# ShuangXieIrene/ssds.pytorch

Hardware: AMD Instinct MI355X
Metric: images/sec (fwd+decode+NMS) SSD-MobileNetV2@512 (higher is better)
Workload: dtype bf16

## Files before the change

### include/ssdk.h

```cpp
#ifndef SSDK_H_
#define SSDK_H_

#include <stddef.h>
#include <stdint.h>

#ifdef __cplusplus
extern "C" {
#endif

#define SSDK_VERSION 245

#define SSDK_MAX_LEVELS 8
#define SSDK_MAX_ANCHORS 16
#define SSDK_MAX_TOPN 1024
#define SSDK_MAX_NDET 1024
#define SSDK_MAX_NMS_N 8192
#define SSDK_MAX_GT 256

enum {
  SSDK_OK = 0,
  SSDK_E_BADARG = -1,
  SSDK_E_WORKSPACE = -2,
  SSDK_E_LAUNCH = -3,
  SSDK_E_NODEVICE = -4
// ... 100 lines not shown
                             int stride, int by_scale, float thr_a, float thr_b, float radius, const void* conf,
                             const void* loc, int dtype, float negpos_ratio, float beta, int loc_loss, void* d_conf,
                             void* d_loc, float* sums, void* workspace, size_t workspace_bytes, void* stream);

int ssdk_map_match(const float* scores, const float* boxes, const float* classes, int B, int D,
                   const float* targets, int G, int num_classes, float conf_threshold, float iou_threshold,
                   long long* keys, unsigned char* tp, int* npos, void* stream);

int ssdk_map_average_precision(const unsigned char* tp_sorted, const long long* seg_offsets, const int* npos,
                               int num_classes, double* ap, void* stream);

enum { SSDK_LAYOUT_NCHW = 0, SSDK_LAYOUT_NHWC = 1 };
typedef struct ssdk_conv_desc {
  const void* x;
  const void* w;
  const float* scale;
  const float* bias;
  const void* residual;
  void* y;
  void* y2;
  int32_t N, Cin, H, W, Cout, k, stride, groups;
  int32_t act, act2, split;
  int32_t dtype;
  int32_t in_layout, out_layout;
  int32_t res_mode;
  const void* w_frag;
} ssdk_conv_desc;
size_t ssdk_weight_frag_bytes(int rows, int K);
size_t ssdk_conv_workspace_bytes(int N, int Cin, int H, int W, int Cout, int k, int stride, int dtype);
int ssdk_conv(const ssdk_conv_desc* desc, void* workspace, size_t workspace_bytes, void* stream);
int ssdk_conv_sequence(const ssdk_conv_desc* descs, int n, void* workspace, size_t workspace_bytes,
                       void* stream);

typedef struct ssdk_mbconv_desc {
  const void* x;
  void* y;
  const void* w_expand;
  const float* scale_expand;
  const float* bias_expand;
  const void* w_dw;
  const void* bias_dw;
  const void* w_project;
  const float* scale_project;
  const float* bias_project;
  int32_t N, H, W, Cin, Chid, Cout, stride, residual, dtype;
  int32_t stem;
  int32_t variant;
  int32_t image_nw;
  const void* w_image;
  size_t w_image_bytes;
} ssdk_mbconv_desc;
int ssdk_mbconv(const ssdk_mbconv_desc* desc, void* stream);
size_t ssdk_mbk_image_bytes(int Cin, int Chid, int Cout, int stride, int out_width, int image_nw, int* nfo);

enum { SSDK_FUSE_SAME = 0, SSDK_FUSE_UP2 = 1, SSDK_FUSE_POOL2 = 2 };
typedef struct ssdk_fuse_desc {
  const void* a;
  const void* b;
  const void* c;
  void* y;
  float w0, w1, w2;
  int32_t mode_b, mode_c;
  int32_t N, H, W, C;
  int32_t hb, wb, hc, wc;
  int32_t dtype;
} ssdk_fuse_desc;
int ssdk_fuse(const ssdk_fuse_desc* desc, void* stream);

int ssdk_preprocess(const void* x, int src_dtype, int src_layout, int N, int H, int W, int C, const float* mean,
                    const float* std, void* y, int dst_dtype, void* stream);

typedef struct ssdk_augment_desc {
  int64_t src_offset;
  int32_t src_h, src_w;
  int32_t crop_x, crop_y, crop_w, crop_h;
  int32_t canvas_w, canvas_h, paste_x, paste_y;
  int32_t flip;
  float color[12];
  float fill[3];
} ssdk_augment_desc;
size_t ssdk_augment_desc_bytes(void);
size_t ssdk_augment_workspace_bytes(int B);
int ssdk_augment(const void* pixels, size_t pixels_bytes, const ssdk_augment_desc* descs_host, int B, int H, int W,
                 const float* mean, const float* std, void* y, int dst_dtype, void* workspace, size_t workspace_bytes,
                 void* stream);

int ssdk_pw_prepare(const float* w32, void* w16, void* wt16, int Cout, int Cin, int dtype, void* stream);
size_t ssdk_pw_stats_workspace_bytes(int B, int K, int M, int HW);
int ssdk_pw_forward_stats(const void* x, const void* a, const float* bias, void* y, float* sums, void* workspace,
                          size_t workspace_bytes, int B, int K, int M, int HW, int dtype, void* stream);
int ssdk_pw_forward(const void* x, const void* a, const float* bias, void* y, int B, int K, int M, int HW, int dtype,
                    void* stream);
size_t ssdk_pw_wgrad_workspace_bytes(int B, int Cout, int Cin, int HW);
int ssdk_pw_wgrad(const void* dy, const void* x, float* dw, void* workspace, size_t workspace_bytes, int B, int Cout, int Cin,
                  int HW, int dtype, void* stream);

int ssdk_im2col3x3(const void* x, void* col, int B, int C, int H, int W, int stride, int dtype, void* stream);
int ssdk_col2im3x3(const void* dcol, void* dx, int B, int C, int H, int W, int stride, int dtype, void* stream);
int ssdk_im2col3x3_folded(const void* x, void* col, int B, int C, int H, int W, int stride, int dtype, void* stream);
int ssdk_col2im3x3_folded(const void* dcol, void* dx, int B, int C, int H, int W, int stride, int dtype, void* stream);

size_t ssdk_stem3x3s2_wgrad_workspace_bytes(int N, int H);
int ssdk_stem3x3s2_fwd(const void* x, const float* w, void* y, int N, int Cin, int H, int W, int Cout, int dtype, void* stream);
int ssdk_stem3x3s2_wgrad(const void* x, const void* dy, float* dw, void* workspace, size_t workspace_bytes, int N, int Cin, int H, int W,
                         int Cout, int dtype, void* stream);

// ... 196 lines not shown
```

### ssds.pytorch_amd/csrc/ssdk_mbk.hip

```cpp
#include "ssdk_common.h"
#include "ssdk_flow_common.h"
#include "ssdk_scan.h"

namespace ssdk {

struct MbkParams {
  const u16* x;
  u16* y;
  const unsigned char* img;
  int N, H, W, Ho, Wo, Cin, Chid, Cout, residual;
  int pairs, halves;
  unsigned items;
  unsigned long long* dbg;
  unsigned wave_mask, pair_mask;
};

template <int KS, int NW, int NCHW, int NFO>
struct MbkGeo {
  static constexpr int NP = (NCHW + 1) / 2;
  static constexpr int PAIR_KB = 2 * KS + NFO;
  static constexpr int MISC_KB = (NCHW * 384 + 1023) / 1024;
  static constexpr int m_be = 0, m_wd = NCHW * 64, m_bd = NCHW * (64 + 288);
  static constexpr int SPB_KB = 2;
  static_assert(NFO * 128 <= SPB_KB * 1024, "projection BN block");
  __host__ __device__ static size_t weights(int halves) { return (size_t)halves * NW * NP * PAIR_KB * 1024; }
  __host__ __device__ static size_t misc_off(int halves) { return weights(halves); }
  __host__ __device__ static size_t spb_off(int halves) { return misc_off(halves) + (size_t)NW * MISC_KB * 1024; }
  __host__ __device__ static size_t bytes(int halves) { return spb_off(halves) + (size_t)halves * SPB_KB * 1024; }
};

template <int S, int NS>
struct MbkItem {
  static constexpr int NXS = NS * S;
  static constexpr int NR = S + 3;
};

template <int S, int NS, int KS, int NW, int NCHW, int NFO>
struct MbkLds {
  using G = MbkGeo<KS, NW, NCHW, NFO>;
  using I = MbkItem<S, NS>;
  static constexpr int FT = 2 * NS * NFO;
  static constexpr int XF = FT % 5 == 0 ? 5 : (FT % 8 == 0 ? 8 : 4);
  static_assert(FT % XF == 0, "exchange rounds");
  static constexpr int xt = 0;
  static constexpr int misc = xt + I::NR * I::NXS * KS * 1024;
  static constexpr int spb = misc + NW * G::MISC_KB * 1024;
  static constexpr int xch = spb + G::SPB_KB * 1024;
  static constexpr int bytes = xch + NW * XF * 1024;
};

__device__ __forceinline__ void mbk_mfma_guard() {
  __builtin_amdgcn_sched_barrier(0);
  asm volatile("s_nop 15\n\ts_nop 3" ::: "memory");
  __builtin_amdgcn_sched_barrier(0);
}
__device__ __forceinline__ void mbk_valu_guard() {
  __builtin_amdgcn_sched_barrier(0);
  asm volatile("s_nop 3" ::: "memory");
  __builtin_amdgcn_sched_barrier(0);
}
__device__ __forceinline__ u32 fl_from_left2(u32 cur, u32 prev) {
  const int old = __builtin_amdgcn_update_dpp(0, (int)prev, 0x121, 0xf, 0xf, true);
  return (u32)__builtin_amdgcn_update_dpp(old, (int)cur, 0x111, 0xf, 0xf, false);
}
__device__ __forceinline__ u32 fl_from_right2(u32 cur, u32 next) {
  const int old = __builtin_amdgcn_update_dpp(0, (int)next, 0x12f, 0xf, 0xf, true);
  return (u32)__builtin_amdgcn_update_dpp(old, (int)cur, 0x101, 0xf, 0xf, false);
}

template <int DT, int S, int NS, int KS, int NW, int NCHW, int NFO, bool DBG = false>
__global__ __launch_bounds__(64 * NW, 2) void mbk_kernel(const MbkParams p) {
  using L = MbkLds<S, NS, KS, NW, NCHW, NFO>;
  using G = MbkGeo<KS, NW, NCHW, NFO>;
  using I = MbkItem<S, NS>;
  constexpr int NR = I::NR, NXS = I::NXS, NE = NR * NXS;
  constexpr int XF = L::XF, FT = L::FT, NP = G::NP, PAIR_KB = G::PAIR_KB;
  constexpr int NO = 2 * NS;
  constexpr bool ODD = (NCHW & 1) != 0;
  constexpr int ROUNDS = FT / XF;
  extern __shared__ __attribute__((aligned(16))) unsigned char smem[];
  const u32 tid = threadIdx.x, lane = tid & 63u;
  const u32 fr = lane & 15u, fg = lane >> 4;
  const int wv = __builtin_amdgcn_readfirstlane((int)(tid >> 6));
  const int Cin = p.Cin, Cout = p.Cout, H = p.H, W = p.W, Ho = p.Ho, Wo = p.Wo;

  const u32 item = blockIdx.x;
  const int half = (int)(item % (u32)p.halves);
  const u32 rem = item / (u32)p.halves;
  const int n = (int)(rem / (u32)p.pairs), rp = (int)(rem % (u32)p.pairs);
  const int oy0 = 2 * rp;
  const int iy0 = S * oy0 - 1;
  const int co_base = half * 16 * NFO;
  const u16* ximg = p.x + (size_t)n * H * W * Cin;
  const bool stamp = p.dbg != nullptr && blockIdx.x == 0 && tid == 0;
  if (stamp) p.dbg[0] = __builtin_readcyclecounter();

  const u32x4* wimg = reinterpret_cast<const u32x4*>(p.img + ((size_t)(half * NW + wv) * NP) * ((size_t)PAIR_KB * 1024)) + lane;
  u32x4 wa[KS], wb[KS];
#pragma unroll
  for (int ks = 0; ks < KS; ++ks) {
    wa[ks] = wimg[(size_t)ks * 64];
    wb[ks] = wimg[(size_t)(KS + ks) * 64];
  }

  for (int e = wv; e < NE; e += NW) {
    const int r = e / NXS, xs = e % NXS;
    int iy = iy0 + r;
    iy = iy < 0 ? 0 : (iy > H - 1 ? H - 1 : iy);
    const int col = S == 1 ? 16 * xs + (int)fr : 2 * (16 * (xs >> 1) + (int)fr) + (xs & 1);
    const u16* src = ximg + ((size_t)iy * W + col) * Cin + fg * 8;
#pragma unroll
    for (int ks = 0; ks < KS; ++ks)
      __builtin_amdgcn_global_load_lds((glb_u8*)(src + ks * 32), (lds_u8*)(smem + L::xt + (e * KS + ks) * 1024), 16, 0, 0);
  }
  {
    const unsigned char* src = p.img + G::misc_off(p.halves) + (size_t)wv * (G::MISC_KB * 1024) + lane * 16;
#pragma unroll
    for (int k = 0; k < G::MISC_KB; ++k)
      __builtin_amdgcn_global_load_lds((glb_u8*)(src + k * 1024), (lds_u8*)(smem + L::misc + (wv * G::MISC_KB + k) * 1024), 16, 0, 0);
  }
  if (wv == 0) {
    const unsigned char* src = p.img + G::spb_off(p.halves) + (size_t)half * (G::SPB_KB * 1024) + lane * 16;
#pragma unroll
    for (int k = 0; k < G::SPB_KB; ++k)
      __builtin_amdgcn_global_load_lds((glb_u8*)(src + k * 1024), (lds_u8*)(smem + L::spb + k * 1024), 16, 0, 0);
  }
  asm volatile("s_waitcnt vmcnt(0)" ::: "memory");
  __syncthreads();
  if (stamp) p.dbg[1] = __builtin_readcyclecounter();

  fl_f2 hi[NR];
#pragma unroll
  for (int r = 0; r < NR; ++r) {
    const float k = ((unsigned)(iy0 + r) < (unsigned)H) ? kFlSixth : 0.f;
    hi[r] = fl_f2{k, k};
  }

  f32x4 yacc[NO][NFO];
#pragma unroll
  for (int o = 0; o < NO; ++o)
#pragma unroll
    for (int f = 0; f < NFO; ++f) yacc[o][f] = f32x4{0.f, 0.f, 0.f, 0.f};

  const unsigned char* xt = smem + L::xt + lane * 16;
  const unsigned char* mc = smem + L::misc + wv * (G::MISC_KB * 1024);

  auto chunk = [&](int c, const u32x4 (&w)[KS], u32 (&dout)[NO][2]) {
    const f32x4 bv = *reinterpret_cast<const f32x4*>(mc + G::m_be + (c * 4 + (int)fg) * 16);
    f32x4 e[NE];
#pragma unroll
    for (int i = 0; i < NE; ++i) e[i] = bv;
#pragma unroll
    for (int ks = 0; ks < KS; ++ks) {
      u32x4 xf[NE];
#pragma unroll
      for (int i = 0; i < NE; ++i) xf[i] = *reinterpret_cast<const u32x4*>(xt + (i * KS + ks) * 1024);
#pragma unroll
      for (int i = 0; i < NE; ++i) e[i] = fl_mfma<DT>(w[ks], xf[i], e[i]);
    }
    uint2 wt[9];
#pragma unroll
    for (int t = 0; t < 9; ++t) wt[t] = *reinterpret_cast<const uint2*>(mc + G::m_wd + ((c * 9 + t) * 4 + (int)fg) * 8);
    const uint2 bdi = *reinterpret_cast<const uint2*>(mc + G::m_bd + (c * 4 + (int)fg) * 8);
    mbk_mfma_guard();
    u32 ew[NR][NXS][2];
#pragma unroll
    for (int r = 0; r < NR; ++r)
#pragma unroll
      for (int xs = 0; xs < NXS; ++xs) {
        ew[r][xs][0] = fl_unit_pack(e[r * NXS + xs][0], e[r * NXS + xs][1], hi[r]);
        ew[r][xs][1] = fl_unit_pack(e[r * NXS + xs][2], e[r * NXS + xs][3], hi[r]);
      }
#pragma unroll
    for (int o = 0; o < 2; ++o)
#pragma unroll
      for (int j = 0; j < NS; ++j) {
        fl_h2 s[2] = {fl_as_h2(bdi.x), fl_as_h2(bdi.y)};
#pragma unroll
        for (int ky = 0; ky < 3; ++ky) {
          const int r = S * o + ky;
          const uint2 w0 = wt[ky * 3], w1 = wt[ky * 3 + 1], w2 = wt[ky * 3 + 2];
#pragma unroll
          for (int wd = 0; wd < 2; ++wd) {
            u32 tl, tc, tr;
            if constexpr (S == 1) {
              tc = ew[r][j][wd];
              tl = j == 0 ? fl_from_left(tc) : fl_from_left2(tc, ew[r][j > 0 ? j - 1 : 0][wd]);
              tr = j == NS - 1 ? fl_from_right(tc) : fl_from_right2(tc, ew[r][j < NS - 1 ? j + 1 : j][wd]);
            } else {
              const u32 odd = ew[r][2 * j + 1][wd];
              tc = ew[r][2 * j][wd];
              tl = j == 0 ? fl_from_left(odd) : fl_from_left2(odd, ew[r][j > 0 ? 2 * j - 1 : 1][wd]);
              tr = odd;
            }
            const u32 ww0 = wd ? w0.y : w0.x, ww1 = wd ? w1.y : w1.x, ww2 = wd ? w2.y : w2.x;
            s[wd] = __builtin_elementwise_fma(fl_as_h2(tl), fl_as_h2(ww0), s[wd]);
            s[wd] = __builtin_elementwise_fma(fl_as_h2(tc), fl_as_h2(ww1), s[wd]);
            if (ky == 2) s[wd] = fl_fma_clamp01(fl_as_h2(tr), fl_as_h2(ww2), s[wd]);
            else s[wd] = __builtin_elementwise_fma(fl_as_h2(tr), fl_as_h2(ww2), s[wd]);
          }
        }
        dout[o * NS + j][0] = fl_as_u32(s[0]);
        dout[o * NS + j][1] = fl_as_u32(s[1]);
      }
  };

  constexpr int FH = NFO / 2;
  for (int t = 0; t < NP; ++t) {
    const u32x4* wp = wimg + (size_t)t * (PAIR_KB * 64);
    const bool last = t == NP - 1;
    const u32x4* wn = wimg + (size_t)(last ? t : t + 1) * (PAIR_KB * 64);
    u32 d0[NO][2], d1[NO][2];
    u32x4 wf0[FH], wf1[NFO - FH];
#pragma unroll
    for (int f = 0; f < FH; ++f) wf0[f] = wp[(size_t)(2 * KS + f) * 64];
    chunk(2 * t, wa, d0);
    __builtin_amdgcn_sched_barrier(0);
    u32x4 na[KS];
#pragma unroll
    for (int ks = 0; ks < KS; ++ks) na[ks] = wn[(size_t)ks * 64];
#pragma unroll
    for (int f = FH; f < NFO; ++f) wf1[f - FH] = wp[(size_t)(2 * KS + f) * 64];
    if (!(ODD && last)) {
      chunk(2 * t + 1, wb, d1);
    } else {
#pragma unroll
      for (int o = 0; o < NO; ++o) d1[o][0] = d1[o][1] = 0u;
    }
    __builtin_amdgcn_sched_barrier(0);
    u32x4 nb[KS];
#pragma unroll
    for (int ks = 0; ks < KS; ++ks) nb[ks] = wn[(size_t)(KS + ks) * 64];
    u32x4 db[NO];
#pragma unroll
    for (int o = 0; o < NO; ++o) db[o] = u32x4{d0[o][0], d0[o][1], d1[o][0], d1[o][1]};
    if constexpr (DBG) {
      if (!((p.pair_mask >> t) & 1u) || !((p.wave_mask >> wv) & 1u)) {
#pragma unroll
        for (int o = 0; o < NO; ++o) db[o] = u32x4{0u, 0u, 0u, 0u};
      }
    }
    mbk_valu_guard();
#pragma unroll
    for (int f = 0; f < NFO; ++f)
#pragma unroll
      for (int o = 0; o < NO; ++o)
        yacc[o][f] = fl_mfma<SSDK_F16>(f < FH ? wf0[f < FH ? f : 0] : wf1[f >= FH ? f - FH : 0], db[o], yacc[o][f]);
    __builtin_amdgcn_sched_barrier(0);
#pragma unroll
    for (int ks = 0; ks < KS; ++ks) {
      wa[ks] = na[ks];
      wb[ks] = nb[ks];
    }
  }
  if (stamp) p.dbg[2] = __builtin_readcyclecounter();

  unsigned char* xb = smem + L::xch;
  const unsigned char* spb = smem + L::spb;
  constexpr int GPW = (XF + NW - 1) / NW;
  uint2 resv[ROUNDS][GPW];
#pragma unroll
  for (int R = 0; R < ROUNDS; ++R)
#pragma unroll
    for (int gg = 0; gg < GPW; ++gg) {
      const int g = wv + gg * NW, q = R * XF + g, oj = q / NFO, f = q % NFO;
      const int oy = oy0 + oj / NS, ox = 16 * (oj % NS) + (int)fr, co = co_base + f * 16 + (int)fg * 4;
      resv[R][gg] = make_uint2(0u, 0u);
      if (S == 1 && p.residual && g < XF && oy < Ho && co < Cout)
        resv[R][gg] = *reinterpret_cast<const uint2*>(ximg + ((size_t)oy * W + ox) * Cin + co);
    }
#pragma unroll
  for (int R = 0; R < ROUNDS; ++R) {
#pragma unroll
    for (int g = 0; g < XF; ++g) {
      const int q = R * XF + g, oj = q / NFO, f = q % NFO;
      *reinterpret_cast<f32x4*>(xb + ((wv * XF + g) * 64 + (int)lane) * 16) = yacc[oj][f];
    }
    __syncthreads();
#pragma unroll
    for (int gg = 0; gg < GPW; ++gg) {
      const int g = wv + gg * NW;
      if (g < XF) {
        const int q = R * XF + g, oj = q / NFO, f = q % NFO;
        f32x4 y = *reinterpret_cast<const f32x4*>(xb + ((0 * XF + g) * 64 + (int)lane) * 16);
#pragma unroll
        for (int w2 = 1; w2 < NW; ++w2) {
          const f32x4 t2 = *reinterpret_cast<const f32x4*>(xb + ((w2 * XF + g) * 64 + (int)lane) * 16);
          y = y + t2;
        }
        const int oy = oy0 + oj / NS, ox = 16 * (oj % NS) + (int)fr;
        const int co = co_base + f * 16 + (int)fg * 4;
        if (oy < Ho && co < Cout) {
          const f32x4 spv = *reinterpret_cast<const f32x4*>(spb + (f * 4 + (int)fg) * 32);
          const f32x4 bpv = *reinterpret_cast<const f32x4*>(spb + (f * 4 + (int)fg) * 32 + 16);
          u32 h01 = fl_pack2<DT>(fmaf(y[0], spv[0], bpv[0]), fmaf(y[1], spv[1], bpv[1]));
          u32 h23 = fl_pack2<DT>(fmaf(y[2], spv[2], bpv[2]), fmaf(y[3], spv[3], bpv[3]));
          if (S == 1 && p.residual) {
            const uint2 xr = resv[R][gg];
            h01 = fl_pack2<DT>(fl_from16<DT>(h01 & 0xffffu) + fl_from16<DT>(xr.x & 0xffffu), fl_from16<DT>(h01 >> 16) + fl_from16<DT>(xr.x >> 16));
            h23 = fl_pack2<DT>(fl_from16<DT>(h23 & 0xffffu) + fl_from16<DT>(xr.y & 0xffffu), fl_from16<DT>(h23 >> 16) + fl_from16<DT>(xr.y >> 16));
          }
          u16* yrow = p.y + (((size_t)n * Ho + oy) * Wo + ox) * Cout;
          *reinterpret_cast<uint2*>(yrow + co) = make_uint2(h01, h23);
        }
      }
    }
    if (R + 1 < ROUNDS) __syncthreads();
  }
  if (stamp) p.dbg[3] = __builtin_readcyclecounter();
}

template <int DT, int S, int NS, int KS, int NW, int NCHW, int NFO, bool DBG = false>
static void mbk_launch(const MbkParams& p, hipStream_t stream) {
  constexpr int lds = MbkLds<S, NS, KS, NW, NCHW, NFO>::bytes;
  static_assert(lds <= 160 * 1024, "LDS");
  (void)hipFuncSetAttribute(reinterpret_cast<const void*>(&mbk_kernel<DT, S, NS, KS, NW, NCHW, NFO, DBG>),
                            hipFuncAttributeMaxDynamicSharedMemorySize, lds);
  hipLaunchKernelGGL((mbk_kernel<DT, S, NS, KS, NW, NCHW, NFO, DBG>), dim3(p.items), dim3(64 * NW), lds, stream, p);
}

constexpr int kMbkNW = 4;
struct MbkInst {
  int s, ns, ks, nchw, nfo;
};
static const MbkInst kMbkInst[] = {{1, 1, 5, 15, 10}, {2, 1, 3, 9, 10}, {1, 2, 2, 6, 4}, {1, 2, 2, 6, 6}, {1, 2, 3, 9, 6},
                                   {2, 2, 1, 3, 4}, {1, 4, 1, 3, 2}};

static int mbk_find(int stride, int Wo, int Cin, int Chid, int Cout, int nw, int* halves) {
  if (nw != kMbkNW || Cin % 32 || Chid % 16 || Cout % 16 || Wo % 16) return -1;
  const int ks = Cin / 32, nch = Chid / 16, nchw = (nch + nw - 1) / nw, ns = Wo / 16;
  for (int i = 0; i < (int)(sizeof(kMbkInst) / sizeof(kMbkInst[0])); ++i) {
    const MbkInst& k = kMbkInst[i];
    if (k.s == stride && k.ns == ns && k.ks == ks && k.nchw == nchw && Cout % (16 * k.nfo) == 0) {
      if (halves) *halves = Cout / (16 * k.nfo);
      return i;
    }
  }
  return -1;
}

static size_t mbk_bytes(int inst, int halves) {
  switch (inst) {
    case 0: return MbkGeo<5, kMbkNW, 15, 10>::bytes(halves);
    case 1: return MbkGeo<3, kMbkNW, 9, 10>::bytes(halves);
    case 2: return MbkGeo<2, kMbkNW, 6, 4>::bytes(halves);
    case 3: return MbkGeo<2, kMbkNW, 6, 6>::bytes(halves);
    case 4: return MbkGeo<3, kMbkNW, 9, 6>::bytes(halves);
    case 5: return MbkGeo<1, kMbkNW, 3, 4>::bytes(halves);
    case 6: return MbkGeo<1, kMbkNW, 3, 2>::bytes(halves);
  }
  return 0;
}

template <int DT>
static void mbk_dispatch(const MbkParams& p, int inst, hipStream_t stream) {
  const bool dbg = p.wave_mask != ~0u || p.pair_mask != ~0u;
  switch (inst) {
    case 0: dbg ? mbk_launch<DT, 1, 1, 5, kMbkNW, 15, 10, true>(p, stream) : mbk_launch<DT, 1, 1, 5, kMbkNW, 15, 10>(p, stream); break;
    case 1: mbk_launch<DT, 2, 1, 3, kMbkNW, 9, 10>(p, stream); break;
    case 2: mbk_launch<DT, 1, 2, 2, kMbkNW, 6, 4>(p, stream); break;
    case 3: mbk_launch<DT, 1, 2, 2, kMbkNW, 6, 6>(p, stream); break;
    case 4: mbk_launch<DT, 1, 2, 3, kMbkNW, 9, 6>(p, stream); break;
    case 5: mbk_launch<DT, 2, 2, 1, kMbkNW, 3, 4>(p, stream); break;
    case 6: mbk_launch<DT, 1, 4, 1, kMbkNW, 3, 2>(p, stream); break;
  }
}

int launch_mbk(const ssdk_mbconv_desc* d, hipStream_t stream) {
  static const int env = getenv("SSDK_MBK") ? atoi(getenv("SSDK_MBK")) : 1;
  const int variant = d->variant;
  if ((!env && variant != 3) || (variant != 0 && variant != 3)) return 1;
  if (d->stem || !d->w_image || d->image_nw < 1 || (d->stride != 1 && d->stride != 2)) return 1;
  const int Ho = (d->H + 2 - 3) / d->stride + 1, Wo = (d->W + 2 - 3) / d->stride + 1;
  if (d->W != Wo * d->stride) return 1;
  int halves = 0;
  const int inst = mbk_find(d->stride, Wo, d->Cin, d->Chid, d->Cout, d->image_nw, &halves);
  if (inst < 0 || (size_t)d->w_image_bytes < mbk_bytes(inst, halves) || ((uintptr_t)d->w_image & 15)) return 1;
  if (env != 1 && variant != 3 && !((env >> (inst + 1)) & 1)) return 1;
  const int pairs = (Ho + 1) / 2;
  const long items = (long)halves * d->N * pairs;
  constexpr int env_min = 256;
  if (items < env_min && variant != 3) return 1;
  MbkParams p;
  p.x = (const u16*)d->x;
  p.y = (u16*)d->y;
  p.img = (const unsigned char*)d->w_image;
  p.N = d->N;
  p.H = d->H;
  p.W = d->W;
  p.Ho = Ho;
  p.Wo = Wo;
  p.Cin = d->Cin;
  p.Chid = d->Chid;
  p.Cout = d->Cout;
  p.residual = d->residual;
  p.pairs = pairs;
  p.halves = halves;
  p.items = (unsigned)items;
  p.dbg = nullptr;
  p.wave_mask = p.pair_mask = ~0u;
  if (const char* m = getenv("SSDK_MBK_MASKS")) {
    unsigned a = ~0u, b = ~0u;
    if (sscanf(m, "%x,%x", &a, &b) == 2) {
      p.wave_mask = a;
      p.pair_mask = b;
    }
  }
  static const int env_dbg = getenv("SSDK_MB_DBG") ? atoi(getenv("SSDK_MB_DBG")) : 0;
  static unsigned long long* dbg_dev = nullptr;
  if (env_dbg) {
    if (!dbg_dev) (void)hipMalloc(&dbg_dev, 8 * sizeof(unsigned long long));
    p.dbg = dbg_dev;
  }
  if (d->dtype == SSDK_BF16) mbk_dispatch<SSDK_BF16>(p, inst, stream);
  else mbk_dispatch<SSDK_F16>(p, inst, stream);
  if (env_dbg) {
    unsigned long long h[4];
    (void)hipStreamSynchronize(stream);
    (void)hipMemcpy(h, dbg_dev, sizeof(h), hipMemcpyDeviceToHost);
    fprintf(stderr, "[mbk dbg] Cin=%d Chid=%d Cout=%d s=%d W=%d items=%ld : setup %llu loop %llu exchange %llu\n", d->Cin, d->Chid,
            d->Cout, d->stride, d->W, items, h[1] - h[0], h[2] - h[1], h[3] - h[2]);
  }
  return 0;
}

}

extern "C" size_t ssdk_mbk_image_bytes(int Cin, int Chid, int Cout, int stride, int Wo, int nw, int* nfo) {
  int halves = 0;
  const int inst = ssdk::mbk_find(stride, Wo, Cin, Chid, Cout, nw, &halves);
  if (inst < 0) return 0;
  if (nfo) *nfo = ssdk::kMbkInst[inst].nfo;
  return ssdk::mbk_bytes(inst, halves);
}
```

### ssds.pytorch_amd/ssds/_native.py

```python
import ctypes
import os
import threading

import torch

_HERE = os.path.dirname(os.path.abspath(__file__))
LIB_PATH = os.path.join(os.path.dirname(_HERE), "csrc", "libssdk.so")

MAX_LEVELS = 8
MAX_ANCHORS = 16
MAX_TOPN = 1024
MAX_NDET = 1024
MAX_NMS_N = 8192
MAX_GT = 256

F32, BF16, F16 = 0, 1, 2
ACT = {"none": 0, "relu": 1, "relu6": 2, "silu": 3, "sigmoid": 4}
_DTYPES = {torch.float32: F32, torch.bfloat16: BF16, torch.float16: F16}
U8 = 3


class Level(ctypes.Structure):
    _fields_ = [
        ("cls", ctypes.c_void_p),
# ... 62 lines not shown
class MbSeDesc(ctypes.Structure):
    _fields_ = [(n, ctypes.c_void_p) for n in (
        "x", "t", "pool_partial", "gate", "y", "residual", "w_dw", "scale_dw", "bias_dw", "w_se1", "b_se1", "w_se2", "b_se2",
        "w_proj", "scale_proj", "bias_proj")] + [(n, ctypes.c_int32) for n in (
            "N", "H", "W", "C", "R", "Cout", "k", "stride", "dtype", "stages")]


class Op(ctypes.Structure):
    _fields_ = [("kind", ctypes.c_int32), ("lane", ctypes.c_int32), ("conv", ConvDesc), ("mb", MbConvDesc),
                ("fuse", FuseDesc), ("stem", StemDesc), ("pool", PoolDesc), ("xpair", XpairDesc), ("mbse", MbSeDesc)]


OP_CONV, OP_MBCONV, OP_FUSE, OP_STEM7, OP_POOL, OP_XPAIR, OP_MBSE = 0, 1, 2, 3, 4, 5, 6
MBSE_DW, MBSE_GATE, MBSE_PROJ = 1, 2, 4
FUSE_SAME, FUSE_UP2, FUSE_POOL2 = 0, 1, 2
NCHW, NHWC = 0, 1


ABI_VERSION = 245


def _load():
    if not os.path.exists(LIB_PATH):
        raise ImportError(
            "libssdk.so not found at {} -- build it first: `python -c 'import __graft_entry__ as g; "
            "g.build()'` or `make -C ssds.pytorch_amd/csrc` (there is no CPU fallback)".format(LIB_PATH)
        )
    lib = ctypes.CDLL(LIB_PATH)
    c = ctypes
    vp, i32, f32, sz = c.c_void_p, c.c_int, c.c_float, c.c_size_t
    lib.ssdk_version.restype = i32
    try:
        have = int(lib.ssdk_version())
    except AttributeError:
        have = 0
    if have < ABI_VERSION:
        raise ImportError("libssdk.so at {} is ABI {} but ssds/_native.py is written for ABI {}: rebuild it "
                          "(`make -C ssds.pytorch_amd/csrc`)".format(LIB_PATH, have, ABI_VERSION))
    lib.ssdk_struct_size.argtypes = [i32]
    lib.ssdk_struct_size.restype = sz
    for which, cls in enumerate((Level, ConvDesc, MbConvDesc, FuseDesc, StemDesc, PoolDesc, XpairDesc, Op)):
        want = lib.ssdk_struct_size(which)
        if want != ctypes.sizeof(cls):
            raise ImportError("libssdk.so at {} was built against another include/ssdk.h: sizeof({}) is {} there, {} in ssds/_native.py"
                              .format(LIB_PATH, cls.__name__, want, ctypes.sizeof(cls)))
    lib.ssdk_last_error.restype = c.c_char_p
    lib.ssdk_abi_check.argtypes = [i32, sz]
    lib.ssdk_abi_check.restype = i32
    if lib.ssdk_abi_check(ABI_VERSION, ctypes.sizeof(Op)) != 0:
        raise ImportError("libssdk.so at {}: {}".format(LIB_PATH, lib.ssdk_last_error().decode()))
    lib.ssdk_last_kernel.restype = c.c_char_p
    lib.ssdk_mbk_image_bytes.argtypes = [i32] * 6 + [c.POINTER(i32)]
    lib.ssdk_mbk_image_bytes.restype = sz
    lib.ssdk_fuse.argtypes = [c.POINTER(FuseDesc), vp]
    lib.ssdk_fuse.restype = i32
    lib.ssdk_pw_prepare.argtypes = [vp, vp, vp, i32, i32, i32, vp]
    lib.ssdk_pw_forward.argtypes = [vp, vp, vp, vp, i32, i32, i32, i32, i32, vp]
    lib.ssdk_pw_stats_workspace_bytes.argtypes = [i32] * 4
    lib.ssdk_pw_stats_workspace_bytes.restype = sz
    lib.ssdk_pw_forward_stats.argtypes = [vp, vp, vp, vp, vp, vp, sz, i32, i32, i32, i32, i32, vp]
    lib.ssdk_pw_forward_stats.restype = i32
    lib.ssdk_bn_act_train_fwd_sums.argtypes = [vp, vp, vp, vp, vp, vp, vp, vp, vp, vp, sz, i32, i32, i32, f32, f32, i32, i32, vp]
    lib.ssdk_bn_act_train_fwd_sums.restype = i32
    lib.ssdk_pw_wgrad_workspace_bytes.argtypes = [i32] * 4
    lib.ssdk_pw_wgrad_workspace_bytes.restype = sz
    lib.ssdk_pw_wgrad.argtypes = [vp, vp, vp, vp, sz, i32, i32, i32, i32, i32, vp]
    lib.ssdk_sgd_step.argtypes = [i32, vp, vp, vp, vp, vp, f32, f32, f32, i32, vp, vp]
    lib.ssdk_sgd_step.restype = i32
    f64 = c.c_double
    lib.ssdk_adam_step.argtypes = [i32, vp, vp, vp, vp, vp, vp, vp, vp, f32, f64, f64, f32, f32, i32, vp, vp]
    lib.ssdk_adam_step.restype = i32
    lib.ssdk_rmsprop_step.argtypes = [i32, vp, vp, vp, vp, vp, vp, vp, f32, f64, f32, f32, f32, vp, vp]
    lib.ssdk_rmsprop_step.restype = i32
    lib.ssdk_im2col3x3.argtypes = [vp, vp, i32, i32, i32, i32, i32, i32, vp]
    lib.ssdk_col2im3x3.argtypes = [vp, vp, i32, i32, i32, i32, i32, i32, vp]
    lib.ssdk_im2col3x3_folded.argtypes = lib.ssdk_col2im3x3_folded.argtypes = [vp, vp, i32, i32, i32, i32, i32, i32, vp]
    lib.ssdk_im2col3x3_folded.restype = lib.ssdk_col2im3x3_folded.restype = i32
    lib.ssdk_stem3x3s2_wgrad_workspace_bytes.argtypes = [i32, i32]
    lib.ssdk_stem3x3s2_wgrad_workspace_bytes.restype = sz
    lib.ssdk_stem3x3s2_fwd.argtypes = [vp, vp, vp, i32, i32, i32, i32, i32, i32, vp]
    lib.ssdk_stem3x3s2_wgrad.argtypes = [vp, vp, vp, vp, sz, i32, i32, i32, i32, i32, i32, vp]
    lib.ssdk_stem3x3s2_fwd.restype = lib.ssdk_stem3x3s2_wgrad.restype = i32
    lib.ssdk_stem7x7s2_wgrad_workspace_bytes.argtypes = [i32] * 4
    lib.ssdk_stem7x7s2_wgrad_workspace_bytes.restype = sz
    lib.ssdk_stem7x7s2_fwd.argtypes = [vp, vp, vp, i32, i32, i32, i32, i32, i32, vp]
    lib.ssdk_stem7x7s2_wgrad.argtypes = [vp, vp, vp, vp, sz, i32, i32, i32, i32, i32, i32, vp]
    lib.ssdk_stem7x7s2_fwd.restype = lib.ssdk_stem7x7s2_wgrad.restype = i32
    lib.ssdk_dwconv5_bwd_weight_workspace_bytes.argtypes = [i32] * 5
    lib.ssdk_dwconv5_bwd_weight_workspace_bytes.restype = sz
    lib.ssdk_dwconv5_fwd.argtypes = lib.ssdk_dwconv5_bwd_data.argtypes = [vp, vp, vp, i32, i32, i32, i32, i32, i32, vp]
    lib.ssdk_dwconv5_bwd_weight.argtypes = [vp, vp, vp, vp, sz, i32, i32, i32, i32, i32, i32, vp]
    lib.ssdk_se_pool_fwd.argtypes = [vp, vp, i32, i32, i32, i32, i32, vp]
    lib.ssdk_se_gate_fwd.argtypes = [vp] * 7 + [i32, i32, i32, vp]
    lib.ssdk_se_scale_fwd.argtypes = lib.ssdk_se_bwd_reduce.argtypes = [vp, vp, vp, i32, i32, i32, i32, i32, vp]
    lib.ssdk_se_gate_bwd_workspace_bytes.argtypes = [i32] * 3
    lib.ssdk_se_gate_bwd_workspace_bytes.restype = sz
    lib.ssdk_se_gate_bwd.argtypes = [vp] * 12 + [sz, i32, i32, i32, vp]
    lib.ssdk_se_bwd_apply.argtypes = [vp, vp, vp, vp, vp, i32, i32, i32, i32, i32, vp]
    for _n in ("ssdk_dwconv5_fwd", "ssdk_dwconv5_bwd_data", "ssdk_dwconv5_bwd_weight", "ssdk_se_pool_fwd", "ssdk_se_gate_fwd",
               "ssdk_se_scale_fwd", "ssdk_se_bwd_reduce", "ssdk_se_gate_bwd", "ssdk_se_bwd_apply"):
        getattr(lib, _n).restype = i32
    lib.ssdk_gconv3x3_train_prepare.argtypes = [vp, vp, vp, i32, i32, i32, vp]
    lib.ssdk_gconv3x3_train_forward.argtypes = [vp, vp, vp, i32, i32, i32, i32, i32, i32, i32, vp]
    lib.ssdk_gconv3x3_train_dgrad.argtypes = [vp, vp, vp, i32, i32, i32, i32, i32, i32, i32, vp]
    lib.ssdk_gconv3x3_train_wgrad_workspace_bytes.argtypes = [i32] * 6
    lib.ssdk_gconv3x3_train_wgrad_workspace_bytes.restype = sz
# ... 126 lines not shown
                                     vp, vp, sz, vp]
    lib.ssdk_conv.argtypes = [c.POINTER(ConvDesc), vp, sz, vp]
    lib.ssdk_conv.restype = i32
    lib.ssdk_conv_sequence.argtypes = [c.POINTER(ConvDesc), i32, vp, sz, vp]
    lib.ssdk_conv_sequence.restype = i32
    lib.ssdk_mbconv.argtypes = [c.POINTER(MbConvDesc), vp]
    lib.ssdk_augment_desc_bytes.restype = sz
    lib.ssdk_augment_desc_bytes.argtypes = []
    if int(lib.ssdk_augment_desc_bytes()) != c.sizeof(AugmentDesc):
        raise ImportError("libssdk.so at {} has sizeof(ssdk_augment_desc) = {} but ssds/_native.py mirrors it with {} bytes: "
                          "rebuild it (`make -C ssds.pytorch_amd/csrc`)".format(LIB_PATH, int(lib.ssdk_augment_desc_bytes()),
                                                                               c.sizeof(AugmentDesc)))
    lib.ssdk_mbse_desc_bytes.restype = sz
    lib.ssdk_mbse_desc_bytes.argtypes = []
    if int(lib.ssdk_mbse_desc_bytes()) != c.sizeof(MbSeDesc):
        raise ImportError("libssdk.so at {} has sizeof(ssdk_mbse_desc) = {} but ssds/_native.py mirrors it with {} bytes: "
                          "rebuild it (`make -C ssds.pytorch_amd/csrc`)".format(LIB_PATH, int(lib.ssdk_mbse_desc_bytes()),
                                                                               c.sizeof(MbSeDesc)))
    lib.ssdk_mbse.argtypes = [c.POINTER(MbSeDesc), vp]
    lib.ssdk_mbse.restype = i32
    lib.ssdk_mbse_pool_tiles.argtypes = [i32] * 4
    lib.ssdk_mbse_pool_tiles.restype = i32
    lib.ssdk_augment_workspace_bytes.restype = sz
    lib.ssdk_augment_workspace_bytes.argtypes = [i32]
    lib.ssdk_augment.argtypes = [vp, sz, c.POINTER(AugmentDesc), i32, i32, i32, c.POINTER(f32), c.POINTER(f32), vp, i32, vp, sz, vp]
    lib.ssdk_augment.restype = i32
    lib.ssdk_mbconv.restype = i32
    lib.ssdk_xpair.argtypes = [c.POINTER(XpairDesc), vp]
    lib.ssdk_xpair.restype = i32
    lib.ssdk_run_ops.argtypes = [c.POINTER(Op), i32, vp, sz, vp]
    lib.ssdk_run_ops.restype = i32
    lib.ssdk_set_profiling.argtypes = [i32]
    lib.ssdk_get_timings.argtypes = [i32, c.POINTER(f32), i32]
    for name in ("ssdk_set_profiling", "ssdk_get_timings", "ssdk_device_info", "ssdk_generate_anchors", "ssdk_decode", "ssdk_nms",
                 "ssdk_decode_nms", "ssdk_match_targets", "ssdk_match_targets_by_scale", "ssdk_conv_bn_act"):
        getattr(lib, name).restype = i32
    return lib


lib = _load()
EXPORTS = ("ssdk_version", "ssdk_struct_size", "ssdk_abi_check", "ssdk_last_error", "ssdk_last_kernel", "ssdk_set_op_profiling", "ssdk_get_op_timings", "ssdk_device_info", "ssdk_generate_anchors",
           "ssdk_decode_workspace_bytes", "ssdk_decode", "ssdk_nms_workspace_bytes", "ssdk_nms",
           "ssdk_decode_nms_workspace_bytes", "ssdk_decode_nms", "ssdk_match_targets",
           "ssdk_match_targets_by_scale", "ssdk_match_loss_workspace_bytes", "ssdk_match_loss",
           "ssdk_match_multibox_loss_workspace_bytes", "ssdk_match_multibox_loss",
           "ssdk_map_match", "ssdk_map_average_precision", "ssdk_set_decode_tail_stream", "ssdk_debug_lds_probe",
           "ssdk_ctx_create", "ssdk_ctx_destroy", "ssdk_ctx_set_tail_stream", "ssdk_ctx_set_side_lane", "ssdk_ctx_set_profiling",
           "ssdk_ctx_get_timings", "ssdk_ctx_set_op_profiling", "ssdk_ctx_get_op_timings", "ssdk_ctx_get_tail_stamps",
           "ssdk_run_ops_ctx", "ssdk_decode_nms_ctx",
           "ssdk_weight_frag_bytes", "ssdk_conv_workspace_bytes", "ssdk_conv", "ssdk_conv_sequence", "ssdk_mbconv", "ssdk_mbk_image_bytes", "ssdk_mbse", "ssdk_mbse_pool_tiles", "ssdk_mbse_desc_bytes", "ssdk_xpair", "ssdk_fuse", "ssdk_preprocess", "ssdk_augment_desc_bytes", "ssdk_augment_workspace_bytes", "ssdk_augment", "ssdk_dwconv_fwd_stats_workspace_bytes", "ssdk_dwconv_fwd_stats", "ssdk_dwconv_affine_supported", "ssdk_dwconv_fwd_affine", "ssdk_dwconv_bwd_weight_affine", "ssdk_bn_act_train_stats", "ssdk_pw_prepare", "ssdk_pw_forward", "ssdk_pw_stats_workspace_bytes", "ssdk_pw_forward_stats", "ssdk_bn_act_train_fwd_sums", "ssdk_pw_wgrad_workspace_bytes", "ssdk_pw_wgrad", "ssdk_im2col3x3", "ssdk_col2im3x3", "ssdk_im2col3x3_folded", "ssdk_col2im3x3_folded", "ssdk_stem3x3s2_wgrad_workspace_bytes", "ssdk_stem3x3s2_fwd", "ssdk_stem3x3s2_wgrad", "ssdk_stem7x7s2_wgrad_workspace_bytes", "ssdk_stem7x7s2_fwd", "ssdk_stem7x7s2_wgrad", "ssdk_dwconv5_bwd_weight_workspace_bytes", "ssdk_dwconv5_fwd", "ssdk_dwconv5_bwd_data", "ssdk_dwconv5_bwd_weight", "ssdk_se_pool_fwd", "ssdk_se_gate_fwd", "ssdk_se_scale_fwd", "ssdk_se_bwd_reduce", "ssdk_se_gate_bwd_workspace_bytes", "ssdk_se_gate_bwd", "ssdk_se_bwd_apply", "ssdk_gconv3x3_train_prepare", "ssdk_gconv3x3_train_forward", "ssdk_gconv3x3_train_dgrad", "ssdk_gconv3x3_train_wgrad_workspace_bytes", "ssdk_gconv3x3_train_wgrad", "ssdk_conv3x3_train_prepare", "ssdk_conv3x3_train_forward", "ssdk_conv3x3_train_dgrad", "ssdk_conv3x3_train_wgrad_workspace_bytes", "ssdk_conv3x3_train_wgrad", "ssdk_pack_conv3x3", "ssdk_pack_conv3x3_dgrad", "ssdk_concat_nchw_to_nhwc", "ssdk_sgd_step", "ssdk_adam_step", "ssdk_rmsprop_step", "ssdk_dwconv_fwd", "ssdk_dwconv_bwd_data",
           "ssdk_dwconv_bwd_weight_workspace_bytes", "ssdk_dwconv_bwd_weight", "ssdk_dwconv_plan", "ssdk_bn_workspace_bytes",
           "ssdk_bn_train_fwd", "ssdk_bn_train_bwd", "ssdk_bn_act_train_fwd", "ssdk_bn_act_train_bwd", "ssdk_bn_sync_local_stats",
           "ssdk_bn_sync_fwd_finalize", "ssdk_bn_act_apply", "ssdk_bn_sync_bwd_local", "ssdk_bn_sync_bwd_apply", "ssdk_conv_stem7", "ssdk_maxpool3x3s2", "ssdk_neck_fuse_fwd", "ssdk_neck_fuse_bwd_workspace_bytes", "ssdk_neck_fuse_bwd",
           "ssdk_maxpool3x3s2_train_fwd", "ssdk_maxpool3x3s2_train_bwd", "ssdk_run_ops", "ssdk_conv_bn_act", "ssdk_set_profiling", "ssdk_get_timings")


class Context(object):

    def __init__(self, device):
        self.device = torch.device(device)
        with torch.cuda.device(self.device):
            self.ptr = lib.ssdk_ctx_create()
        if not self.ptr:
            raise SsdkError("ssdk_ctx_create failed: " + lib.ssdk_last_error().decode())
        self.ptr = ctypes.c_void_p(self.ptr)

    def __del__(self):
        try:
            if getattr(self, "ptr", None):
                lib.ssdk_ctx_destroy(self.ptr)
                self.ptr = None
        except Exception:
            pass

    def _call(self, fn, *a):
        with torch.cuda.device(self.device):
            return fn(self.ptr, *a)

    def set_tail_stream(self, stream):
        check(self._call(lib.ssdk_ctx_set_tail_stream, ctypes.c_void_p(stream.cuda_stream) if stream is not None else None),
              "ctx_set_tail_stream")

    def set_side_lane(self, on):
        self.side_user = None if on is None else bool(on)
        self.side_auto = False
        check(self._call(lib.ssdk_ctx_set_side_lane, -1 if on is None else int(bool(on))), "ctx_set_side_lane")

    def auto_side_lane(self):
        if getattr(self, "side_user", None) is not None or getattr(self, "side_auto", False):
            return
        if os.environ.get("SSDK_SIDE_STREAM", "") == "0":
            return
        check(self._call(lib.ssdk_ctx_set_side_lane, 1), "ctx_set_side_lane")
        self.side_auto = True

    def set_profiling(self, on):
        check(self._call(lib.ssdk_ctx_set_profiling, 2 if on == 2 else (1 if on else 0)), "ctx_set_profiling")

    def timings_ms(self, back=0):
        ms = (ctypes.c_float * 3)()
        check(self._call(lib.ssdk_ctx_get_timings, int(back), ms, 3), "ctx_get_timings")
        return float(ms[0]), float(ms[1]), float(ms[2])

    def set_op_profiling(self, on):
        check(self._call(lib.ssdk_ctx_set_op_profiling, 1 if on else 0), "ctx_set_op_profiling")

    def op_timings(self):
# ... 121 lines not shown
```

Before: 64090.

## Run three workgroups per CU for small MBConv instances by overlapping LDS regions

Adds a WG3 template mode in which the exchange buffer reuses the LDS space of the input tile and constants, guarded by an extra barrier, so three workgroups fit in a CU's 160 KB. In that mode the expand MFMAs are software-pipelined with a short fragment window to cut register pressure, and the depthwise accumulation is restructured row by row, using an SGPR-operand packed multiply-clamp. It is enabled by default only for instance 6, with an env override, and an occupancy query API is added. The cost is an extra __syncthreads, a possibly smaller exchange round size, and register limits tightened by launch bounds of 3.

Result: no change. 64100 (median of 2 runs) (+0.0%).

```diff
diff --git a/include/ssdk.h b/include/ssdk.h
--- a/include/ssdk.h
+++ b/include/ssdk.h
@@ -176,6 +176,7 @@
 } ssdk_mbconv_desc;
 int ssdk_mbconv(const ssdk_mbconv_desc* desc, void* stream);
 size_t ssdk_mbk_image_bytes(int Cin, int Chid, int Cout, int stride, int out_width, int image_nw, int* nfo);
+int ssdk_mbk_occupancy(int Cin, int Chid, int Cout, int stride, int out_width, int dtype);
 
 enum { SSDK_FUSE_SAME = 0, SSDK_FUSE_UP2 = 1, SSDK_FUSE_POOL2 = 2 };
 typedef struct ssdk_fuse_desc {
diff --git a/ssds.pytorch_amd/csrc/ssdk_mbk.hip b/ssds.pytorch_amd/csrc/ssdk_mbk.hip
--- a/ssds.pytorch_amd/csrc/ssdk_mbk.hip
+++ b/ssds.pytorch_amd/csrc/ssdk_mbk.hip
@@ -35,18 +35,23 @@
   static constexpr int NR = S + 3;
 };
 
-template <int S, int NS, int KS, int NW, int NCHW, int NFO>
+template <int S, int NS, int KS, int NW, int NCHW, int NFO, int WG3 = 2>
 struct MbkLds {
   using G = MbkGeo<KS, NW, NCHW, NFO>;
   using I = MbkItem<S, NS>;
   static constexpr int FT = 2 * NS * NFO;
-  static constexpr int XF = FT % 5 == 0 ? 5 : (FT % 8 == 0 ? 8 : 4);
+  static constexpr int dead = (I::NR * I::NXS * KS + NW * G::MISC_KB) * 1024;
+  static constexpr int XF2 = FT % 5 == 0 ? 5 : (FT % 8 == 0 ? 8 : 4);
+  static constexpr int XF = WG3 == 3 && (dead > NW * XF2 * 1024 ? dead : NW * XF2 * 1024) + G::SPB_KB * 1024 > 53 * 1024 ? 4 : XF2;
   static_assert(FT % XF == 0, "exchange rounds");
   static constexpr int xt = 0;
   static constexpr int misc = xt + I::NR * I::NXS * KS * 1024;
-  static constexpr int spb = misc + NW * G::MISC_KB * 1024;
-  static constexpr int xch = spb + G::SPB_KB * 1024;
-  static constexpr int bytes = xch + NW * XF * 1024;
+  static constexpr int spb = WG3 == 3 ? (dead > NW * XF * 1024 ? dead : NW * XF * 1024) : dead;
+  static constexpr int xch = WG3 == 3 ? 0 : spb + G::SPB_KB * 1024;
+  static constexpr int bytes = WG3 == 3 ? spb + G::SPB_KB * 1024 : xch + NW * XF * 1024;
+  static_assert(misc + NW * G::MISC_KB * 1024 == dead, "x tile and constants are one region");
+  static_assert(WG3 == 2 || WG3 == 3, "workgroups per CU");
+  static_assert(WG3 == 2 || bytes <= 53 * 1024, "three workgroups share the 160 KB of a CU");
 };
 
 __device__ __forceinline__ void mbk_mfma_guard() {
@@ -59,6 +64,12 @@
   asm volatile("s_nop 3" ::: "memory");
   __builtin_amdgcn_sched_barrier(0);
 }
+__device__ __forceinline__ u32 mbk_unit_pack_s(float a, float b, unsigned long long k) {
+  const fl_f2 v = {a, b};
+  fl_f2 r;
+  asm("v_pk_mul_f32 %0, %1, %2 clamp" : "=v"(r) : "v"(v), "s"(k));
+  return __builtin_bit_cast(u32, __builtin_amdgcn_cvt_pkrtz(r[0], r[1]));
+}
 __device__ __forceinline__ u32 fl_from_left2(u32 cur, u32 prev) {
   const int old = __builtin_amdgcn_update_dpp(0, (int)prev, 0x121, 0xf, 0xf, true);
   return (u32)__builtin_amdgcn_update_dpp(old, (int)cur, 0x111, 0xf, 0xf, false);
@@ -68,9 +79,9 @@
   return (u32)__builtin_amdgcn_update_dpp(old, (int)cur, 0x101, 0xf, 0xf, false);
 }
 
-template <int DT, int S, int NS, int KS, int NW, int NCHW, int NFO, bool DBG = false>
-__global__ __launch_bounds__(64 * NW, 2) void mbk_kernel(const MbkParams p) {
-  using L = MbkLds<S, NS, KS, NW, NCHW, NFO>;
+template <int DT, int S, int NS, int KS, int NW, int NCHW, int NFO, int WG3 = 2, bool DBG = false>
+__global__ __launch_bounds__(64 * NW, WG3) void mbk_kernel(const MbkParams p) {
+  using L = MbkLds<S, NS, KS, NW, NCHW, NFO, WG3>;
   using G = MbkGeo<KS, NW, NCHW, NFO>;
   using I = MbkItem<S, NS>;
   constexpr int NR = I::NR, NXS = I::NXS, NE = NR * NXS;
@@ -135,6 +146,12 @@
     const float k = ((unsigned)(iy0 + r) < (unsigned)H) ? kFlSixth : 0.f;
     hi[r] = fl_f2{k, k};
   }
+  unsigned long long his[NR];
+#pragma unroll
+  for (int r = 0; r < NR; ++r) {
+    const u32 k = ((unsigned)(iy0 + r) < (unsigned)H) ? __builtin_bit_cast(u32, kFlSixth) : 0u;
+    his[r] = ((unsigned long long)k << 32) | k;
+  }
 
   f32x4 yacc[NO][NFO];
 #pragma unroll
@@ -145,32 +162,119 @@
   const unsigned char* xt = smem + L::xt + lane * 16;
   const unsigned char* mc = smem + L::misc + wv * (G::MISC_KB * 1024);
 
+  auto taps = [&](const u32 (&er)[NXS][2], int j, int wd, u32& tl, u32& tc, u32& tr) {
+    if constexpr (S == 1) {
+      tc = er[j][wd];
+      tl = j == 0 ? fl_from_left(tc) : fl_from_left2(tc, er[j > 0 ? j - 1 : 0][wd]);
+      tr = j == NS - 1 ? fl_from_right(tc) : fl_from_right2(tc, er[j < NS - 1 ? j + 1 : j][wd]);
+    } else {
+      const u32 odd = er[2 * j + 1][wd];
+      tc = er[2 * j][wd];
+      tl = j == 0 ? fl_from_left(odd) : fl_from_left2(odd, er[j > 0 ? 2 * j - 1 : 1][wd]);
+      tr = odd;
+    }
+  };
   auto chunk = [&](int c, const u32x4 (&w)[KS], u32 (&dout)[NO][2]) {
     const f32x4 bv = *reinterpret_cast<const f32x4*>(mc + G::m_be + (c * 4 + (int)fg) * 16);
-    f32x4 e[NE];
-#pragma unroll
-    for (int i = 0; i < NE; ++i) e[i] = bv;
-#pragma unroll
-    for (int ks = 0; ks < KS; ++ks) {
-      u32x4 xf[NE];
-#pragma unroll
-      for (int i = 0; i < NE; ++i) xf[i] = *reinterpret_cast<const u32x4*>(xt + (i * KS + ks) * 1024);
-#pragma unroll
-      for (int i = 0; i < NE; ++i) e[i] = fl_mfma<DT>(w[ks], xf[i], e[i]);
-    }
     uint2 wt[9];
-#pragma unroll
-    for (int t = 0; t < 9; ++t) wt[t] = *reinterpret_cast<const uint2*>(mc + G::m_wd + ((c * 9 + t) * 4 + (int)fg) * 8);
-    const uint2 bdi = *reinterpret_cast<const uint2*>(mc + G::m_bd + (c * 4 + (int)fg) * 8);
-    mbk_mfma_guard();
+    uint2 bdi;
     u32 ew[NR][NXS][2];
-#pragma unroll
-    for (int r = 0; r < NR; ++r)
-#pragma unroll
-      for (int xs = 0; xs < NXS; ++xs) {
-        ew[r][xs][0] = fl_unit_pack(e[r * NXS + xs][0], e[r * NXS + xs][1], hi[r]);
-        ew[r][xs][1] = fl_unit_pack(e[r * NXS + xs][2], e[r * NXS + xs][3], hi[r]);
-      }
+    if constexpr (WG3 == 3) {
+      constexpr int D = (3 + KS) / KS, P = 2;
+      static_assert(D * KS >= 4 && D < NE && P <= NE, "independent MFMAs between a fragment's last MFMA and its pack");
+      f32x4 e[D + 1];
+      u32x4 xf[P][KS];
+      auto request = [&](int i) {
+        if (i < NE) {
+#pragma unroll
+          for (int ks = 0; ks < KS; ++ks) xf[i % P][ks] = *reinterpret_cast<const u32x4*>(xt + (i * KS + ks) * 1024);
+        }
+      };
+      auto expand = [&](int i) {
+        f32x4 a = bv;
+#pragma unroll
+        for (int ks = 0; ks < KS; ++ks) a = fl_mfma<DT>(w[ks], xf[i % P][ks], a);
+        e[i % (D + 1)] = a;
+        request(i + P);
+      };
+#pragma unroll
+      for (int i = 0; i < P; ++i) request(i);
+#pragma unroll
+      for (int i = 0; i < D; ++i) {
+        expand(i);
+        __builtin_amdgcn_sched_barrier(0);
+      }
+#pragma unroll
+      for (int i = 0; i < NE; ++i) {
+        if (i + D < NE) {
+          expand(i + D);
+          __builtin_amdgcn_sched_barrier(0);
+        } else if (i + D == NE) {
+          bdi = *reinterpret_cast<const uint2*>(mc + G::m_bd + (c * 4 + (int)fg) * 8);
+          mbk_mfma_guard();
+        }
+        const f32x4 a = e[i % (D + 1)];
+        ew[i / NXS][i % NXS][0] = mbk_unit_pack_s(a[0], a[1], his[i / NXS]);
+        ew[i / NXS][i % NXS][1] = mbk_unit_pack_s(a[2], a[3], his[i / NXS]);
+        if (i + D < NE) __builtin_amdgcn_sched_barrier(0);
+      }
+      fl_h2 s[NO][2];
+#pragma unroll
+      for (int r = 0; r < NR; ++r) {
+#pragma unroll
+        for (int o = 0; o < 2; ++o) {
+          const int ky = r - S * o;
+          if (ky < 0 || ky > 2) continue;
+          uint2 wk[3];
+#pragma unroll
+          for (int kx = 0; kx < 3; ++kx) wk[kx] = *reinterpret_cast<const uint2*>(mc + G::m_wd + ((c * 9 + ky * 3 + kx) * 4 + (int)fg) * 8);
+          const uint2 w0 = wk[0], w1 = wk[1], w2 = wk[2];
+#pragma unroll
+          for (int j = 0; j < NS; ++j)
+#pragma unroll
+            for (int wd = 0; wd < 2; ++wd) {
+              u32 tl, tc, tr;
+              taps(ew[r], j, wd, tl, tc, tr);
+              const u32 ww0 = wd ? w0.y : w0.x, ww1 = wd ? w1.y : w1.x, ww2 = wd ? w2.y : w2.x;
+              fl_h2 a = ky == 0 ? fl_as_h2(wd ? bdi.y : bdi.x) : s[o * NS + j][wd];
+              a = __builtin_elementwise_fma(fl_as_h2(tl), fl_as_h2(ww0), a);
+              a = __builtin_elementwise_fma(fl_as_h2(tc), fl_as_h2(ww1), a);
+              if (ky == 2) a = fl_fma_clamp01(fl_as_h2(tr), fl_as_h2(ww2), a);
+              else a = __builtin_elementwise_fma(fl_as_h2(tr), fl_as_h2(ww2), a);
+              s[o * NS + j][wd] = a;
+            }
+        }
+      }
+#pragma unroll
+      for (int q = 0; q < NO; ++q) {
+        dout[q][0] = fl_as_u32(s[q][0]);
+        dout[q][1] = fl_as_u32(s[q][1]);
+      }
+      return;
+    } else {
+      f32x4 e[NE];
+#pragma unroll
+      for (int i = 0; i < NE; ++i) e[i] = bv;
+#pragma unroll
+      for (int ks = 0; ks < KS; ++ks) {
+        u32x4 xf[NE];
+#pragma unroll
+        for (int i = 0; i < NE; ++i) xf[i] = *reinterpret_cast<const u32x4*>(xt + (i * KS + ks) * 1024);
+#pragma unroll
+        for (int i = 0; i < NE; ++i) e[i] = fl_mfma<DT>(w[ks], xf[i], e[i]);
+      }
+#pragma unroll
+      for (int t = 0; t < 9; ++t) wt[t] = *reinterpret_cast<const uint2*>(mc + G::m_wd + ((c * 9 + t) * 4 + (int)fg) * 8);
+      bdi = *reinterpret_cast<const uint2*>(mc + G::m_bd + (c * 4 + (int)fg) * 8);
+      mbk_mfma_guard();
+#pragma unroll
+      for (int r = 0; r < NR; ++r)
+#pragma unroll
+        for (int xs = 0; xs < NXS; ++xs) {
+          ew[r][xs][0] = fl_unit_pack(e[r * NXS + xs][0], e[r * NXS + xs][1], hi[r]);
+          ew[r][xs][1] = fl_unit_pack(e[r * NXS + xs][2], e[r * NXS + xs][3], hi[r]);
+        }
+    }
 #pragma unroll
     for (int o = 0; o < 2; ++o)
 #pragma unroll
@@ -183,16 +287,7 @@
 #pragma unroll
           for (int wd = 0; wd < 2; ++wd) {
             u32 tl, tc, tr;
-            if constexpr (S == 1) {
-              tc = ew[r][j][wd];
-              tl = j == 0 ? fl_from_left(tc) : fl_from_left2(tc, ew[r][j > 0 ? j - 1 : 0][wd]);
-              tr = j == NS - 1 ? fl_from_right(tc) : fl_from_right2(tc, ew[r][j < NS - 1 ? j + 1 : j][wd]);
-            } else {
-              const u32 odd = ew[r][2 * j + 1][wd];
-              tc = ew[r][2 * j][wd];
-              tl = j == 0 ? fl_from_left(odd) : fl_from_left2(odd, ew[r][j > 0 ? 2 * j - 1 : 1][wd]);
-              tr = odd;
-            }
+            taps(ew[r], j, wd, tl, tc, tr);
             const u32 ww0 = wd ? w0.y : w0.x, ww1 = wd ? w1.y : w1.x, ww2 = wd ? w2.y : w2.x;
             s[wd] = __builtin_elementwise_fma(fl_as_h2(tl), fl_as_h2(ww0), s[wd]);
             s[wd] = __builtin_elementwise_fma(fl_as_h2(tc), fl_as_h2(ww1), s[wd]);
@@ -255,6 +350,7 @@
   }
   if (stamp) p.dbg[2] = __builtin_readcyclecounter();
 
+  if constexpr (WG3 == 3) __syncthreads();
   unsigned char* xb = smem + L::xch;
   const unsigned char* spb = smem + L::spb;
   constexpr int GPW = (XF + NW - 1) / NW;
@@ -310,13 +406,18 @@
   if (stamp) p.dbg[3] = __builtin_readcyclecounter();
 }
 
-template <int DT, int S, int NS, int KS, int NW, int NCHW, int NFO, bool DBG = false>
-static void mbk_launch(const MbkParams& p, hipStream_t stream) {
-  constexpr int lds = MbkLds<S, NS, KS, NW, NCHW, NFO>::bytes;
+template <int DT, int S, int NS, int KS, int NW, int NCHW, int NFO, int WG3 = 2, bool DBG = false>
+static int mbk_launch(const MbkParams* p, hipStream_t stream) {
+  constexpr int lds = MbkLds<S, NS, KS, NW, NCHW, NFO, WG3>::bytes;
   static_assert(lds <= 160 * 1024, "LDS");
-  (void)hipFuncSetAttribute(reinterpret_cast<const void*>(&mbk_kernel<DT, S, NS, KS, NW, NCHW, NFO, DBG>),
-                            hipFuncAttributeMaxDynamicSharedMemorySize, lds);
-  hipLaunchKernelGGL((mbk_kernel<DT, S, NS, KS, NW, NCHW, NFO, DBG>), dim3(p.items), dim3(64 * NW), lds, stream, p);
+  const auto kernel = &mbk_kernel<DT, S, NS, KS, NW, NCHW, NFO, WG3, DBG>;
+  (void)hipFuncSetAttribute(reinterpret_cast<const void*>(kernel), hipFuncAttributeMaxDynamicSharedMemorySize, lds);
+  if (!p) {
+    int wgs = 0;
+    return hipOccupancyMaxActiveBlocksPerMultiprocessor(&wgs, kernel, 64 * NW, lds) == hipSuccess ? wgs : -1;
+  }
+  hipLaunchKernelGGL(kernel, dim3(p->items), dim3(64 * NW), lds, stream, *p);
+  return 0;
 }
 
 constexpr int kMbkNW = 4;
@@ -352,18 +453,28 @@
   return 0;
 }
 
+static const bool kMbkHas3[] = {false, false, true, false, false, true, true};
+static const int kMbkWg3[] = {2, 2, 2, 2, 2, 2, 3};
+static int mbk_wg3(int inst) {
+  static const int env = getenv("SSDK_MBK_WG3") ? atoi(getenv("SSDK_MBK_WG3")) : 1;
+  if (!env || !kMbkHas3[inst]) return 2;
+  return env == 2 ? 3 : kMbkWg3[inst];
+}
+
 template <int DT>
-static void mbk_dispatch(const MbkParams& p, int inst, hipStream_t stream) {
-  const bool dbg = p.wave_mask != ~0u || p.pair_mask != ~0u;
+static int mbk_dispatch(const MbkParams* p, int inst, hipStream_t stream) {
+  const bool dbg = p && (p->wave_mask != ~0u || p->pair_mask != ~0u);
+  const bool w3 = mbk_wg3(inst) == 3;
   switch (inst) {
-    case 0: dbg ? mbk_launch<DT, 1, 1, 5, kMbkNW, 15, 10, true>(p, stream) : mbk_launch<DT, 1, 1, 5, kMbkNW, 15, 10>(p, stream); break;
-    case 1: mbk_launch<DT, 2, 1, 3, kMbkNW, 9, 10>(p, stream); break;
-    case 2: mbk_launch<DT, 1, 2, 2, kMbkNW, 6, 4>(p, stream); break;
-    case 3: mbk_launch<DT, 1, 2, 2, kMbkNW, 6, 6>(p, stream); break;
-    case 4: mbk_launch<DT, 1, 2, 3, kMbkNW, 9, 6>(p, stream); break;
-    case 5: mbk_launch<DT, 2, 2, 1, kMbkNW, 3, 4>(p, stream); break;
-    case 6: mbk_launch<DT, 1, 4, 1, kMbkNW, 3, 2>(p, stream); break;
-  }
+    case 0: return dbg ? mbk_launch<DT, 1, 1, 5, kMbkNW, 15, 10, 2, true>(p, stream) : mbk_launch<DT, 1, 1, 5, kMbkNW, 15, 10>(p, stream);
+    case 1: return mbk_launch<DT, 2, 1, 3, kMbkNW, 9, 10>(p, stream);
+    case 2: return w3 ? mbk_launch<DT, 1, 2, 2, kMbkNW, 6, 4, 3>(p, stream) : mbk_launch<DT, 1, 2, 2, kMbkNW, 6, 4>(p, stream);
+    case 3: return mbk_launch<DT, 1, 2, 2, kMbkNW, 6, 6>(p, stream);
+    case 4: return mbk_launch<DT, 1, 2, 3, kMbkNW, 9, 6>(p, stream);
+    case 5: return w3 ? mbk_launch<DT, 2, 2, 1, kMbkNW, 3, 4, 3>(p, stream) : mbk_launch<DT, 2, 2, 1, kMbkNW, 3, 4>(p, stream);
+    case 6: return w3 ? mbk_launch<DT, 1, 4, 1, kMbkNW, 3, 2, 3>(p, stream) : mbk_launch<DT, 1, 4, 1, kMbkNW, 3, 2>(p, stream);
+  }
+  return -1;
 }
 
 int launch_mbk(const ssdk_mbconv_desc* d, hipStream_t stream) {
@@ -412,8 +523,8 @@
     if (!dbg_dev) (void)hipMalloc(&dbg_dev, 8 * sizeof(unsigned long long));
     p.dbg = dbg_dev;
   }
-  if (d->dtype == SSDK_BF16) mbk_dispatch<SSDK_BF16>(p, inst, stream);
-  else mbk_dispatch<SSDK_F16>(p, inst, stream);
+  if (d->dtype == SSDK_BF16) mbk_dispatch<SSDK_BF16>(&p, inst, stream);
+  else mbk_dispatch<SSDK_F16>(&p, inst, stream);
   if (env_dbg) {
     unsigned long long h[4];
     (void)hipStreamSynchronize(stream);
@@ -433,3 +544,9 @@
   if (nfo) *nfo = ssdk::kMbkInst[inst].nfo;
   return ssdk::mbk_bytes(inst, halves);
 }
+
+extern "C" int ssdk_mbk_occupancy(int Cin, int Chid, int Cout, int stride, int Wo, int dtype) {
+  const int inst = ssdk::mbk_find(stride, Wo, Cin, Chid, Cout, ssdk::kMbkNW, nullptr);
+  if (inst < 0 || (dtype != SSDK_BF16 && dtype != SSDK_F16)) return -1;
+  return dtype == SSDK_BF16 ? ssdk::mbk_dispatch<SSDK_BF16>(nullptr, inst, nullptr) : ssdk::mbk_dispatch<SSDK_F16>(nullptr, inst, nullptr);
+}
diff --git a/ssds.pytorch_amd/ssds/_native.py b/ssds.pytorch_amd/ssds/_native.py
--- a/ssds.pytorch_amd/ssds/_native.py
+++ b/ssds.pytorch_amd/ssds/_native.py
@@ -138,6 +138,11 @@
     lib.ssdk_last_kernel.restype = c.c_char_p
     lib.ssdk_mbk_image_bytes.argtypes = [i32] * 6 + [c.POINTER(i32)]
     lib.ssdk_mbk_image_bytes.restype = sz
+    try:
+        lib.ssdk_mbk_occupancy.argtypes = [i32] * 6
+    except AttributeError:
+        raise ImportError("libssdk.so at {} has no ssdk_mbk_occupancy: rebuild it (`make -C ssds.pytorch_amd/csrc`)".format(LIB_PATH))
+    lib.ssdk_mbk_occupancy.restype = i32
     lib.ssdk_fuse.argtypes = [c.POINTER(FuseDesc), vp]
     lib.ssdk_fuse.restype = i32
     lib.ssdk_pw_prepare.argtypes = [vp, vp, vp, i32, i32, i32, vp]
@@ -370,7 +375,7 @@
            "ssdk_dwconv_bwd_weight_workspace_bytes", "ssdk_dwconv_bwd_weight", "ssdk_dwconv_plan", "ssdk_bn_workspace_bytes",
            "ssdk_bn_train_fwd", "ssdk_bn_train_bwd", "ssdk_bn_act_train_fwd", "ssdk_bn_act_train_bwd", "ssdk_bn_sync_local_stats",
            "ssdk_bn_sync_fwd_finalize", "ssdk_bn_act_apply", "ssdk_bn_sync_bwd_local", "ssdk_bn_sync_bwd_apply", "ssdk_conv_stem7", "ssdk_maxpool3x3s2", "ssdk_neck_fuse_fwd", "ssdk_neck_fuse_bwd_workspace_bytes", "ssdk_neck_fuse_bwd",
-           "ssdk_maxpool3x3s2_train_fwd", "ssdk_maxpool3x3s2_train_bwd", "ssdk_run_ops", "ssdk_conv_bn_act", "ssdk_set_profiling", "ssdk_get_timings")
+           "ssdk_maxpool3x3s2_train_fwd", "ssdk_maxpool3x3s2_train_bwd", "ssdk_mbk_occupancy", "ssdk_run_ops", "ssdk_conv_bn_act", "ssdk_set_profiling", "ssdk_get_timings")
 
 
 class Context(object):
```
